# SKA-INAF/caesar-yolo

Hardware: AMD Instinct MI355X
Metric: 512x512 tiles/sec over 16k x 16k FITS (higher is better)
Workload: dtype f16

## Files before the change

caesar_yolo_amd/csrc/conv_igemm.hip:

```cpp
#include "cy_kernels.h"
#include <cmath>
#include <cstdlib>
#include <cstring>
#include <vector>

namespace cy {

typedef _Float16 f16;
typedef f16 f16x8 __attribute__((ext_vector_type(8)));
typedef f16 f16x4 __attribute__((ext_vector_type(4)));
typedef float f32x4 __attribute__((ext_vector_type(4)));
typedef unsigned int u32x4 __attribute__((ext_vector_type(4)));
typedef unsigned int u32x2 __attribute__((ext_vector_type(2)));

#define CY_OOB 0xFFFFFF00u
#define CY_WAIT_VM(N) asm volatile("s_waitcnt vmcnt(%0)" ::"n"(N) : "memory")

#ifndef CY_STAMPS_ENABLED
#define CY_STAMPS_ENABLED 0
#endif
__device__ unsigned long long g_stamps[8];
constexpr int WG_STAMP_SLOTS = 4096;
__device__ unsigned long long g_wg_stamps[WG_STAMP_SLOTS * 4];
__device__ __forceinline__ unsigned long long stamp_now() {
// ... 2649 lines not shown
        u32x4 x2[4][MI][2];
#pragma unroll
        for (int g = 0; g < 4; ++g) {
            float bv[16];
#pragma unroll
            for (int j = 0; j < 4; ++j) {
                const f32x4 t = *reinterpret_cast<const f32x4*>(bias1_lds + g * 64 + fq * 16 + j * 4);
                bv[j * 4] = t[0]; bv[j * 4 + 1] = t[1]; bv[j * 4 + 2] = t[2]; bv[j * 4 + 3] = t[3];
            }
#pragma unroll
            for (int mi = 0; mi < MI; ++mi) {
                float v[16];
                bias_act16(acc[g * 4][mi], acc[g * 4 + 1][mi], acc[g * 4 + 2][mi], acc[g * 4 + 3][mi], bv, a.act != 0, v);
                f16x8 h0, h1;
#pragma unroll
                for (int j = 0; j < 8; ++j) { h0[j] = (f16)v[j]; h1[j] = (f16)v[8 + j]; }
                x2[g][mi][0] = __builtin_bit_cast(u32x4, h0); x2[g][mi][1] = __builtin_bit_cast(u32x4, h1);
            }
        }
#pragma unroll
        for (int ni = 0; ni < NB * 4; ++ni)
#pragma unroll
            for (int mi = 0; mi < MI; ++mi) acc[ni][mi] = f32x4{0.f, 0.f, 0.f, 0.f};
        CY_WAIT_VM(0);
        __builtin_amdgcn_s_barrier();
#pragma unroll
        for (int c2 = 0; c2 < 4; ++c2) compute_x(c2, x2[c2]);
#pragma unroll
        for (int g = 0; g < NB; ++g) {
            const int cbase = g * 64 + fq * 16;
            if (cbase >= pad64(a.cout2)) continue;
            float bv[16];
#pragma unroll
            for (int j = 0; j < 4; ++j) {
                const f32x4 t = *reinterpret_cast<const f32x4*>(bias2_lds + g * 64 + fq * 16 + j * 4);
                bv[j * 4] = t[0]; bv[j * 4 + 1] = t[1]; bv[j * 4 + 2] = t[2]; bv[j * 4 + 3] = t[3];
            }
#pragma unroll
            for (int mi = 0; mi < MI; ++mi) {
                const int m = m0 + (wave * MI + mi) * 16 + fr;
                if (m >= M) continue;
                const int b = m / HoWo, r = m - b * HoWo;
                const long opix = (long)b * a.out_bs + a.out_ro + r;
                float v[16];
                bias_act16(acc[g * 4][mi], acc[g * 4 + 1][mi], acc[g * 4 + 2][mi], acc[g * 4 + 3][mi], bv, a.act2 != 0, v);
                f16* dst = reinterpret_cast<f16*>(a.out2) + opix * a.out2_ct + a.out2_coff + cbase;
                if (cbase + 16 <= a.cout2) {
                    f16x8 o0, o1;
#pragma unroll
                    for (int j = 0; j < 8; ++j) { o0[j] = (f16)v[j]; o1[j] = (f16)v[8 + j]; }
                    *reinterpret_cast<f16x8*>(dst) = o0;
                    *reinterpret_cast<f16x8*>(dst + 8) = o1;
                } else {
#pragma unroll
                    for (int j = 0; j < 16; ++j)
                        if (cbase + j < a.cout2) dst[j] = (f16)v[j];
                }
            }
        }
        return;
    }
#pragma unroll
    for (int g = 0; g < NB; ++g) {
        const int cbase = n0 + g * 64 + fq * 16;
        if (cbase >= pad64(a.Cout)) continue;
        float bv[16];
#pragma unroll
        for (int j = 0; j < 4; ++j) {
            const f32x4 t = *reinterpret_cast<const f32x4*>(bias_lds + g * 64 + fq * 16 + j * 4);
            bv[j * 4] = t[0]; bv[j * 4 + 1] = t[1]; bv[j * 4 + 2] = t[2]; bv[j * 4 + 3] = t[3];
        }
        float sc[SPLIT ? 16 : 1];
        if constexpr (SPLIT) {
#pragma unroll
            for (int j = 0; j < 16; ++j) sc[j] = a.oscale[cbase + j];
        }
#pragma unroll
        for (int mi = 0; mi < MI; ++mi) {
            const int m = m0 + (wave * MI + mi) * 16 + fr;
            if (m >= M) continue;
            const int b = m / HoWo, r = m - b * HoWo;
            const long opix = (long)b * a.out_bs + a.out_ro + r;
            float v[16];
            if constexpr (SPLIT) {
                scale_bias_act16(acc[g * 4][mi], acc[g * 4 + 1][mi], acc[g * 4 + 2][mi], acc[g * 4 + 3][mi], bv, sc, a.act != 0, v);
                f16* dst = reinterpret_cast<f16*>(a.out) + opix * a.out_ct + a.out_coff + cbase;
                const f16* rp = a.res ? reinterpret_cast<const f16*>(a.res) + (long)m * a.res_ct + a.res_coff + cbase : nullptr;
                if (cbase + 16 <= a.Cout) {
                    if (rp) {
                        const f16x8 r0v = *reinterpret_cast<const f16x8*>(rp), r1v = *reinterpret_cast<const f16x8*>(rp + 8);
                        const f16x8 q0v = *reinterpret_cast<const f16x8*>(rp + a.res_lo), q1v = *reinterpret_cast<const f16x8*>(rp + a.res_lo + 8);
#pragma unroll
                        for (int j = 0; j < 8; ++j) { v[j] += (float)r0v[j] + (float)q0v[j]; v[8 + j] += (float)r1v[j] + (float)q1v[j]; }
                    }
                    store_split16(dst, a.out_lo, v);
                } else {
#pragma unroll
                    for (int j = 0; j < 16; ++j) {
                        if (cbase + j >= a.Cout) continue;
                        float t = v[j];
                        if (rp) t += (float)rp[j] + (float)rp[a.res_lo + j];
                        store_split1(dst + j, a.out_lo, t);
                    }
                }
                continue;
            }
            bias_act16(acc[g * 4][mi], acc[g * 4 + 1][mi], acc[g * 4 + 2][mi], acc[g * 4 + 3][mi], bv, a.act != 0, v);
            if (cbase + 16 <= a.Cout) {
                f16* dst = reinterpret_cast<f16*>(a.out) + opix * a.out_ct + a.out_coff + cbase;
                if (a.res) {
                    const f16* rp = reinterpret_cast<const f16*>(a.res) + (long)m * a.res_ct + a.res_coff + cbase;
                    const f16x8 r0v = *reinterpret_cast<const f16x8*>(rp), r1v = *reinterpret_cast<const f16x8*>(rp + 8);
#pragma unroll
                    for (int j = 0; j < 8; ++j) { v[j] += (float)r0v[j]; v[8 + j] += (float)r1v[j]; }
                }
                f16x8 o0, o1;
#pragma unroll
                for (int j = 0; j < 8; ++j) { o0[j] = (f16)v[j]; o1[j] = (f16)v[8 + j]; }
                *reinterpret_cast<f16x8*>(dst) = o0;
                *reinterpret_cast<f16x8*>(dst + 8) = o1;
            } else {
#pragma unroll
                for (int j = 0; j < 16; ++j) {
                    const int c = cbase + j;
                    if (c >= a.Cout) continue;
                    float t = v[j];
                    if (a.res) t += (float)(reinterpret_cast<const f16*>(a.res)[(long)m * a.res_ct + a.res_coff + c]);
                    reinterpret_cast<f16*>(a.out)[opix * a.out_ct + a.out_coff + c] = (f16)t;
                }
            }
        }
    }
    if (stamps && tid == 0) {
        unsigned long long* rec = g_wg_stamps + (size_t)(blockIdx.x % WG_STAMP_SLOTS) * 4;
        rec[0] = t_loop - t_entry; rec[1] = t_epi - t_loop; rec[2] = stamp_real() - t_epi; rec[3] = c_epi - c_loop;
    }
}

template <int NB, int MI, int RING, bool K3, bool SPLIT = false, int NDW = 8, bool FUSE2 = false>
static hipError_t launch_direct(const ConvArgs& a, hipStream_t s) {
    constexpr int BN = 64 * NB, BM = 8 * MI * 16;
    const size_t lds = (FUSE2 ? 4 : RING) * BN * 128 + 2048;
    static bool attr_set = false;
    if (!attr_set) {
        hipFuncSetAttribute(reinterpret_cast<const void*>(conv1x1_direct_kernel<NB, MI, RING, K3, SPLIT, NDW, FUSE2>), hipFuncAttributeMaxDynamicSharedMemorySize, (int)lds);
        attr_set = true;
    }
    const int M = a.B * a.Ho * a.Wo;
    const int blocks = ((M + BM - 1) / BM) * ((pad64(a.Cout) + BN - 1) / BN);
    hipLaunchKernelGGL((conv1x1_direct_kernel<NB, MI, RING, K3, SPLIT, NDW, FUSE2>), dim3(blocks), dim3(512), lds, s, a);
    return hipGetLastError();
}

template <int WM, int RING, int PB = 2>
static hipError_t launch_halo(const ConvArgs& a, hipStream_t s) {
    constexpr int TH = 4 * WM, NT = WM * 128;
    constexpr int PR = (TH + 2) * 18, NWI = (PR + 7) / 8, NW = NT / 64, PROUNDS = (NWI + NW - 1) / NW;
    const size_t lds = PB * PROUNDS * NW * 1024 + RING * 128 * 128;
    static bool attr_set = false;
    if (!attr_set) {
        hipFuncSetAttribute(reinterpret_cast<const void*>(conv3x3_halo_kernel<WM, RING, PB>), hipFuncAttributeMaxDynamicSharedMemorySize, (int)lds);
        attr_set = true;
    }
    const int blocks = a.B * ((a.Hi + TH - 1) / TH) * ((a.Wi + 15) / 16) * ((pad64(a.Cout) + 127) / 128);
    hipLaunchKernelGGL((conv3x3_halo_kernel<WM, RING, PB>), dim3(blocks), dim3(NT), lds, s, a);
    return hipGetLastError();
}

template <typename T, int WM, int WN, int MI, int NSTAGE = 2, bool SPLIT = false>
static hipError_t launch_t(const ConvArgs& a, hipStream_t s) {
    constexpr int BM = WM * MI * 16, BN = WN * 64;
    const int M = a.B * a.Ho * a.Wo;
    const int ntm = (M + BM - 1) / BM, ntn = (pad64(a.Cout) + BN - 1) / BN;
    const size_t lds = NSTAGE * (BM + BN) * 128;
    static bool attr_set = false;
    if (!attr_set) {
        hipFuncSetAttribute(reinterpret_cast<const void*>(conv_igemm_kernel<T, WM, WN, MI, NSTAGE, SPLIT>),
                            hipFuncAttributeMaxDynamicSharedMemorySize, (int)lds);
        attr_set = true;
    }
    hipLaunchKernelGGL((conv_igemm_kernel<T, WM, WN, MI, NSTAGE, SPLIT>), dim3(ntm * ntn), dim3(WM * WN * 64), lds, s, a);
    return hipGetLastError();
}

static int head_rows(const ConvArgs& a) { const int c = a.Cout < 16 ? a.Cout : 16; const int g = (c + 3) / 4; return 16 * (g < 4 ? g : 4); }
static bool head_direct(const ConvArgs& a, int passes) {
    if (!env_knob("CY_HEAD_DIRECT", 1)) return false;
    if (!(a.k == 1 && a.s == 1 && a.c1 == 0 && !a.up0 && a.Cin >= 64 && a.Cin % 64 == 0 && a.c0 == a.Cin && pad64(a.Cout) == 64 && a.Ho == a.Hi && a.Wo == a.Wi))
        return false;
    if (a.out_f32 ? (a.res || a.act) : (a.out_bs != a.Ho * a.Wo || a.out_ro != 0 || !env_knob("CY_NARROW_DIRECT", 1))) return false;
    return (size_t)passes * (a.Cin / 64) * head_rows(a) * 128 <= 65536;
}
template <bool SPLIT>
static hipError_t launch_head(const ConvArgs& a, hipStream_t s) {
    const int nrows = head_rows(a);
    const size_t lds = (size_t)(SPLIT ? a.split : 1) * (a.Cin / 64) * nrows * 128 + (a.Cout == 64 && a.out_f32 ? 4 * 32 * 68 * 4 : 0);
    static bool attr_set = false;
    if (!attr_set) {
        hipFuncSetAttribute(reinterpret_cast<const void*>(head1x1_kernel<SPLIT>), hipFuncAttributeMaxDynamicSharedMemorySize, 65536 + 4 * 32 * 68 * 4);
        attr_set = true;
    }
    const long M = (long)a.B * a.Ho * a.Wo;
    const long wgs = (M + 127) / 128;
    hipLaunchKernelGGL((head1x1_kernel<SPLIT>), dim3((unsigned)(wgs < 512 ? wgs : 512)), dim3(256), lds, s, a, nrows);
    return hipGetLastError();
}

static int head_pair_pitch(int rowlen) { int tp = rowlen; while (tp % 8 != 4) ++tp; return tp; }
static size_t head_pair_lds(Precision p, const ConvArgs& a, const ConvArgs& b) {
    const size_t pa = p == PREC_F16X3 ? a.split : 1, pb = p == PREC_F16X3 ? b.split : 1;
    return pa * (a.Cin / 64) * 64 * 128 + pb * (b.Cin / 64) * head_rows(b) * 128 + (size_t)8 * 16 * head_pair_pitch(a.out_ct) * 4;
}
bool head_pair_ok(Precision p, const ConvArgs& a, const ConvArgs& b) {
    if (p == PREC_F32 || !env_knob("CY_HEAD_PAIR", 1)) return false;
    if (conv_variant(p, a) != CONV_HEAD_1X1 || conv_variant(p, b) != CONV_HEAD_1X1) return false;
    if (a.B != b.B || a.Ho != b.Ho || a.Wo != b.Wo || a.out != b.out || a.out_ct != b.out_ct || a.out_bs != b.out_bs || a.out_ro != b.out_ro) return false;
    if (a.out_coff != 0 || a.Cout != 64 || b.out_coff != 64 || b.Cout < 1 || b.Cout != a.out_ct - 64) return false;
    return head_pair_lds(p, a, b) <= 128 * 1024;
}
hipError_t launch_head_pair(Precision p, const ConvArgs& a, const ConvArgs& b, hipStream_t s) {
    const size_t lds = head_pair_lds(p, a, b);
    static bool attr_set = false;
    if (!attr_set) {
        hipFuncSetAttribute(reinterpret_cast<const void*>(head1x1_pair_kernel<false>), hipFuncAttributeMaxDynamicSharedMemorySize, 128 * 1024);
        hipFuncSetAttribute(reinterpret_cast<const void*>(head1x1_pair_kernel<true>), hipFuncAttributeMaxDynamicSharedMemorySize, 128 * 1024);
        attr_set = true;
    }
    const long M = (long)a.B * a.Ho * a.Wo;
    const long wgs = (M + 255) / 256;
    const unsigned grid = (unsigned)(wgs < 256 ? wgs : 256);
    if (p == PREC_F16X3) hipLaunchKernelGGL((head1x1_pair_kernel<true>), dim3(grid), dim3(512), lds, s, a, b, head_rows(b), head_pair_pitch(a.out_ct));
    else hipLaunchKernelGGL((head1x1_pair_kernel<false>), dim3(grid), dim3(512), lds, s, a, b, head_rows(b), head_pair_pitch(a.out_ct));
    return hipGetLastError();
}

static const char* const kVariantNames[CONV_NUM_VARIANTS] = {
    "conv_igemm_kernel<2,2,4> generic 128x128", "conv_igemm_kernel<4,1,2> generic 128x64",
    "conv3x3_halo2_kernel 3x3 s1 16x16px x128ch (halo<2,2> for odd slab counts)", "conv3x3_pp_kernel<2> 3x3 s1 16x16px x64ch",
    "conv3x3_pp_kernel<4> 3x3 s1 16x16px x128ch", "conv3x3_halo_kernel<4,*> 3x3 s1 16x16px x128ch",
    "conv3x3_c64_kernel<64|32> 3x3 s1 persistent, Cin 64 or 32", "conv_igemm_kernel<4,2,4,3> generic 256x128, 3-slab ring",
    "conv3x3_wide_kernel 3x3 s1 16x32px x128ch, K slabs of 32",
    "conv1x1_direct_kernel<4,2> 1x1 256px x256ch, pixels to regs", "conv1x1_direct_kernel<2,2> 1x1 256px x128ch, pixels to regs",
    "conv3x3_wide_kernel<WN=1> 3x3 s1 16x32px x64ch", "conv3x3_wide_kernel<dual> 3x3 s1 2 images x 16x16px x128ch",
    "conv3x3_widep_kernel<strip> 3x3 s1 512 flattened px x128ch, persistent",
    "head1x1_kernel detect-head output 1x1, weights stationary in LDS, fp32 rows"};
const char* conv_variant_name(int v) { return v >= 0 && v < CONV_NUM_VARIANTS ? kVariantNames[v] : "?"; }

static bool s2_direct() { static const int v = getenv("CY_S2_DIRECT") ? atoi(getenv("CY_S2_DIRECT")) : 1; return v != 0; }

bool batch_invariant() { const char* e = getenv("CY_BATCH_INVARIANT"); return !e || atoi(e) != 0; }

static int conv_variant_x3(const ConvArgs& a) {
    const bool narrow = pad64(a.Cout) <= 64;
    if (a.k == 3 && a.s == 1 && a.c1 == 0 && !a.up0 && !a.out_f32 && a.Cin % 64 == 0 && a.wgt32 && a.out_bs == a.Ho * a.Wo && a.out_ro == 0) {
        const int wpad = (a.Wi + 31) / 32 * 32;
        const bool fits = (wpad - a.Wi) * 8 <= a.Wi;
        if (narrow && a.Wi % 32 == 0) return CONV_WIDE_64;
        if (narrow && a.Cin >= 128 && env_knob("CY_STRIP", 1) && strip_small(a) && strip_fits(a)) return CONV_STRIP_128;
        if (!narrow && env_knob("CY_STRIP", 1) && strip_fits(a) && strip_cover(a.Hi, a.Wi) + 0.04 < wide2d_cover(a.Hi, a.Wi)) return CONV_STRIP_128;
        if (!narrow && fits) return CONV_WIDE_128;
        if (!narrow && a.Wi <= 16 && a.Wi >= 14) return CONV_WIDE_DUAL;
    }
    if (!a.out_f32 && a.Cin % 64 == 0 && !narrow &&
        ((a.k == 1 && a.s == 1 && (a.c1 == 0 || a.c0 % 64 == 0)) || (a.k == 3 && a.s == 2 && a.c1 == 0 && !a.up0)))
        return pad64(a.Cout) >= 256 ? CONV_DIRECT_256 : CONV_DIRECT_128;
    if (head_direct(a, a.split)) return CONV_HEAD_1X1;
    return narrow ? CONV_GENERIC_64 : CONV_GENERIC_128;
}

int conv_variant(Precision p, const ConvArgs& a) {
    if (p == PREC_F16X3) return conv_variant_x3(a);
    const bool narrow = pad64(a.Cout) <= 64;
    const long Bv = batch_invariant() && a.B < 256 ? 256 : a.B;
    if (p == PREC_F16 && a.k == 3 && a.s == 1 && a.c1 == 0 && !a.up0 && !a.out_f32 && a.Cin == 32 && narrow && a.wgt32 &&
        a.out_bs == a.Ho * a.Wo && a.out_ro == 0)
        return CONV_C64_PERSIST;
    if (p == PREC_F16 && a.k == 3 && a.s == 1 && a.c1 == 0 && !a.up0 && !a.out_f32 && a.Cin % 64 == 0 &&
        a.out_bs == a.Ho * a.Wo && a.out_ro == 0) {
        static const int force = getenv("CY_HALO_WM") ? atoi(getenv("CY_HALO_WM")) : 0;
        static const int wide64 = getenv("CY_WIDE64") ? atoi(getenv("CY_WIDE64")) : 1;
        if (narrow && wide64 && a.wgt32 && a.Cin >= 128 && a.Wi % 32 == 0 && force == 0 &&
            Bv * ((a.Hi + 15) / 16) * (a.Wi / 32) >= 256)
            return CONV_WIDE_64;
        if (narrow && force == 0 && a.wgt32 && a.Cin >= 128 && env_knob("CY_STRIP", 1) && strip_small(a) && strip_fits(a)) return CONV_STRIP_128;
        if (narrow && a.Cin == 64 && force != 8) return force == 9 ? CONV_GENERIC_64 : CONV_C64_PERSIST;
        if (narrow) return force == 9 ? CONV_GENERIC_64 : CONV_PP_64;
        if (force == 5) return CONV_PP_128;
        if (force == 4 || force == 43) return CONV_HALO16_128;
        static const int wide = getenv("CY_WIDE") ? atoi(getenv("CY_WIDE")) : 1;
        const int strip = env_knob("CY_STRIP", 1);
        if (wide && strip && a.wgt32 && strip_fits(a) && strip_cover(a.Hi, a.Wi) + 0.04 < wide2d_cover(a.Hi, a.Wi) &&
            (strip > 1 || strip_small(a) || Bv * (long)(a.Hi + 1) * (a.Wi + 1) / 512 * ((pad64(a.Cout) + 127) / 128) >= 200))
            return CONV_STRIP_128;
        const int wpad = (a.Wi + 31) / 32 * 32;
        if (wide && a.wgt32 && (wpad - a.Wi) * 8 <= a.Wi) return CONV_WIDE_128;
        const int dual = getenv("CY_WIDE_DUAL") ? atoi(getenv("CY_WIDE_DUAL")) : 1;
        if (wide && dual && a.wgt32 && a.Wi <= 16 && a.Wi >= 14 &&
            ((Bv + 1) / 2) * ((a.Hi + 15) / 16) * ((pad64(a.Cout) + 127) / 128) >= (dual > 1 ? 1 : 224))
            return CONV_WIDE_DUAL;
        return CONV_HALO8_128;
    }
    if (p == PREC_F16 && head_direct(a, 1)) return CONV_HEAD_1X1;
    if (narrow) return CONV_GENERIC_64;
    if (p == PREC_F16 && !a.out_f32 && a.Cin % 64 == 0 &&
        ((a.k == 1 && a.s == 1 && (a.c1 == 0 || a.c0 % 64 == 0)) || (a.k == 3 && a.s == 2 && a.c1 == 0 && !a.up0 && (a.Cin >= 128 || pad64(a.Cout) < 256) && s2_direct()))) {
        const char* e = getenv("CY_DIRECT_MIN_BLOCKS");
        const long min_blocks = e ? atol(e) : 256;
        static const int bn_force = getenv("CY_DIRECT_BN") ? atoi(getenv("CY_DIRECT_BN")) : 0;
        const int bn = bn_force == 128 && a.k == 1 ? 128 : (pad64(a.Cout) >= 256 ? 256 : 128);
        const long blocks = ((Bv * a.Ho * a.Wo + 255) / 256) * ((pad64(a.Cout) + bn - 1) / bn);
        if (min_blocks >= 0 && blocks >= min_blocks) return bn == 256 ? CONV_DIRECT_256 : CONV_DIRECT_128;
    }
    static const int big = getenv("CY_BIG") ? atoi(getenv("CY_BIG")) : 1;
    const long M = Bv * a.Ho * a.Wo;
    if (p == PREC_F16 && big && (M / 256) * ((pad64(a.Cout) + 127) / 128) >= big * 256) return CONV_GENERIC_BIG;
    return CONV_GENERIC_128;
}

hipError_t launch_conv(Precision p, const ConvArgs& a, hipStream_t s) {
    if (p == PREC_F16X3) {
        if ((a.split != 2 && a.split != 3) || !a.oscale) return hipErrorInvalidValue;
        switch (conv_variant_x3(a)) {
            case CONV_WIDE_128:
                if (env_knob("CY_X3_PERSIST", 0) && a.Cout % 16 == 0) return launch_widep(a, s);
                return launch_wide<2, false, 2, true>(a, s);
            case CONV_STRIP_128: return launch_strip(a, s);
            case CONV_WIDE_64: return launch_wide<1, false, 2, true>(a, s);
            case CONV_WIDE_DUAL: return launch_wide<2, true, 2, true>(a, s);
            case CONV_DIRECT_256: return a.k == 3 ? launch_direct<4, 2, 3, true, true>(a, s) : launch_direct<4, 2, 3, false, true>(a, s);
            case CONV_DIRECT_128: return a.k == 3 ? launch_direct<2, 4, 2, true, true>(a, s) : launch_direct<2, 2, 2, false, true>(a, s);
            case CONV_HEAD_1X1: return launch_head<true>(a, s);
            case CONV_GENERIC_64: return launch_t<f16, 4, 1, 2, 2, true>(a, s);
            default: return launch_t<f16, 2, 2, 4, 2, true>(a, s);
        }
    }
    switch (conv_variant(p, a)) {
        case CONV_C64_PERSIST: return a.Cin == 32 ? launch_c64<32>(a, s) : launch_c64<64>(a, s);
        case CONV_PP_64: return launch_pp<2>(a, s);
        case CONV_PP_128: { ConvArgs b2 = a; b2.dbg = dev_knob("CY_DBG", 0); return launch_pp<4>(b2, s); }
        case CONV_HALO16_128: return (getenv("CY_HALO_WM") && atoi(getenv("CY_HALO_WM")) == 43) ? launch_halo<4, 3>(a, s) : launch_halo<4, 2>(a, s);
        case CONV_HALO8_128: {
            ConvArgs b2 = a; b2.dbg = dev_knob("CY_DBG", 0);
            static const int v = getenv("CY_HALO_V") ? atoi(getenv("CY_HALO_V")) : 2;
            if (v == 2 && (a.Cin / 64) % 2 == 0) return launch_halo2(b2, s);
            return v == 1 ? launch_halo<2, 3, 1>(b2, s) : launch_halo<2, 2>(b2, s);
        }
        case CONV_GENERIC_BIG: return launch_t<f16, 4, 2, 4, 3>(a, s);
        case CONV_WIDE_128: {
            static const int tps = getenv("CY_WIDE_TPS") ? atoi(getenv("CY_WIDE_TPS")) : 2;
            ConvArgs b2 = a; b2.dbg = dev_knob("CY_DBG", 0);
            if (const int mf = env_knob("CY_WIDE_MFMA", 16); mf >= 32) return mf == 33 ? launch_wide32<1>(b2, s) : launch_wide32<0>(b2, s);
            const int wp = env_knob("CY_WIDE_PERSIST", 1);
            const long patches = (long)a.B * ((a.Wi + 31) / 32) * ((a.Hi + 15) / 16) * ((pad64(a.Cout) + 127) / 128);
            if (wp && tps == 2 && a.Cout % 16 == 0 && (wp > 1 || (patches >= 512 && a.Cin <= 128))) return launch_widep(b2, s);
            if (tps == 2 && env_knob("CY_WIDE_SCHED", 0)) return launch_wide<2, false, 2, false, 1>(b2, s);
            return tps == 3 ? launch_wide<2, false, 3>(b2, s) : launch_wide<2>(b2, s);
        }
        case CONV_STRIP_128: return launch_strip(a, s);
        case CONV_WIDE_64: return launch_wide<1>(a, s);
        case CONV_WIDE_DUAL: return launch_wide<2, true>(a, s);
        case CONV_DIRECT_256: {
            ConvArgs a2 = a; a2.dbg = dev_knob("CY_DBG", 0);
            static const int v256 = getenv("CY_D256_V") ? atoi(getenv("CY_D256_V")) : 0;
            if (a.k != 3 && v256 > 0 && a.Cin <= v256) return launch_direct<4, 1, 2, false>(a, s);
            static const int ndw = env_knob("CY_DIRECT_NDW", 0);
            if (a.wgt2 && pad64(a.Cout) == 256 && a.c1 == 0 && !a.res && !a.out_f32)
                return a.k == 3 ? launch_direct<4, 2, 3, true, false, 4, true>(a2, s) : launch_direct<4, 2, 3, false, false, 8, true>(a2, s);
            if (a.k == 3) return ndw == 8 ? launch_direct<4, 2, 3, true>(a2, s) : launch_direct<4, 2, 3, true, false, 4>(a2, s);
            return ndw == 4 ? launch_direct<4, 2, 3, false, false, 4>(a2, s) : launch_direct<4, 2, 3, false>(a2, s);
        }
        case CONV_DIRECT_128:
            if (a.k != 3 && !(getenv("CY_D128_V") && atoi(getenv("CY_D128_V")) == 0)) return launch_direct<2, 2, 2, false>(a, s);
            return a.k == 3 ? launch_direct<2, 4, 2, true>(a, s) : launch_direct<2, 2, 4, false>(a, s);
        case CONV_HEAD_1X1: return launch_head<false>(a, s);
        case CONV_GENERIC_64: return p == PREC_F16 ? launch_t<f16, 4, 1, 2>(a, s) : launch_t<float, 4, 1, 2>(a, s);
        default: return p == PREC_F16 ? launch_t<f16, 2, 2, 4>(a, s) : launch_t<float, 2, 2, 4>(a, s);
    }
}

void debug_read_wg_stamps(unsigned long long* out, int n) {
    hipDeviceSynchronize();
    hipMemcpyFromSymbol(out, HIP_SYMBOL(g_wg_stamps), (size_t)(n < WG_STAMP_SLOTS ? n : WG_STAMP_SLOTS) * 4 * sizeof(unsigned long long));
}

void debug_read_stamps(unsigned long long* out8, bool reset) {
    hipDeviceSynchronize();
    hipMemcpyFromSymbol(out8, HIP_SYMBOL(g_stamps), 8 * sizeof(unsigned long long));
    if (CY_STAMPS_ENABLED && out8[6] == 0) {
        static unsigned long long rec[WG_STAMP_SLOTS * 4];
        hipMemcpyFromSymbol(rec, HIP_SYMBOL(g_wg_stamps), sizeof(rec));
        for (int i = 0; i < WG_STAMP_SLOTS; ++i)
            if (rec[i * 4 + 1]) { out8[6] += 1; for (int j = 0; j < 4; ++j) out8[j] += rec[i * 4 + j]; }
        out8[4] = out8[0] + out8[1] + out8[2] + out8[3];
        if (reset) { memset(rec, 0, sizeof(rec)); hipMemcpyToSymbol(HIP_SYMBOL(g_wg_stamps), rec, sizeof(rec)); }
    }
    if (reset) { unsigned long long z[8] = {0}; hipMemcpyToSymbol(HIP_SYMBOL(g_stamps), z, sizeof(z)); }
}

size_t packed_weight_bytes(Precision p, int cout, int cin, int k, int chunk_bytes) {
    const int epb = chunk_bytes / (p == PREC_F16 ? 2 : 4);
    return (size_t)((cin + epb - 1) / epb) * k * k * pad128(cout) * chunk_bytes;
}

void pack_weights(Precision p, const float* W, int cout, int cin, int k, void* dst, int chunk_bytes) {
    const int taps = k * k, cp = pad128(cout), epb = chunk_bytes / (p == PREC_F16 ? 2 : 4), chunks = (cin + epb - 1) / epb;
    memset(dst, 0, packed_weight_bytes(p, cout, cin, k, chunk_bytes));
    for (int row = 0; row < cp; ++row) {
        const int blk = row >> 6, ni = (row >> 4) & 3, rr = row & 15;
        const int n = blk * 64 + (rr >> 2) * 16 + ni * 4 + (rr & 3);
        if (n >= cout) continue;
        for (int t = 0; t < taps; ++t)
            for (int c = 0; c < cin; ++c) {
                const float v = W[((size_t)n * cin + c) * taps + t];
                const size_t o = (((size_t)(c / epb) * taps + t) * cp + row) * epb + (c % epb);
                if (p == PREC_F16) reinterpret_cast<f16*>(dst)[o] = (f16)v;
                else reinterpret_cast<float*>(dst)[o] = v;
            }
    }
    (void)chunks;
}

void pack_weights_fused2(const float* W2, int cout2, int cin2, void* dst) {
    std::vector<float> perm((size_t)cout2 * cin2);
    for (int n = 0; n < cout2; ++n)
        for (int p = 0; p < cin2; ++p) {
            const int c = p >> 6, kk = (p >> 5) & 1, q = (p >> 3) & 3, j = p & 7;
            perm[(size_t)n * cin2 + p] = W2[(size_t)n * cin2 + 64 * c + 16 * q + 8 * kk + j];
        }
    pack_weights(PREC_F16, perm.data(), cout2, cin2, 1, dst);
}

int x3_passes(const float* W, int cout, int cin, int k, const float* scale) {
    const size_t per = (size_t)cin * k * k;
    for (int n = 0; n < cout; ++n) {
        const float sc = scale ? scale[n] : 1.0f;
        if (!(sc != 0.0f) || !std::isfinite(sc)) return 3;
        for (size_t i = 0; i < per; ++i) {
            const float w = W[(size_t)n * per + i];
            const f16 h = (f16)(w / sc);
            if (!((float)h * sc == w)) return 3;
        }
    }
    return 2;
}

size_t packed_weight_bytes_x3(int cout, int cin, int k, int chunk_bytes, int passes) {
    const int epb = chunk_bytes / 2;
    return packed_weight_bytes(PREC_F16, cout, passes * ((cin + epb - 1) / epb * epb), k, chunk_bytes);
}

void pack_weights_x3(const float* W, int cout, int cin, int k, void* dst, float* oscale, int chunk_bytes, int passes, const float* scale) {
    const int taps = k * k, epb = chunk_bytes / 2, cinp = (cin + epb - 1) / epb * epb, cp = pad128(cout);
    memset(dst, 0, packed_weight_bytes_x3(cout, cin, k, chunk_bytes, passes));
    for (int i = 0; i < cp; ++i) oscale[i] = 1.0f;
    f16* o = reinterpret_cast<f16*>(dst);
    for (int row = 0; row < cp; ++row) {
        const int blk = row >> 6, ni = (row >> 4) & 3, rr = row & 15;
        const int n = blk * 64 + (rr >> 2) * 16 + ni * 4 + (rr & 3);
        if (n >= cout) continue;
        if (passes == 2) {
            const float sc = scale ? scale[n] : 1.0f;
            oscale[n] = sc;
            for (int t = 0; t < taps; ++t)
                for (int c = 0; c < cin; ++c) {
                    const f16 h = (f16)(W[((size_t)n * cin + c) * taps + t] / sc);
                    for (int pass = 0; pass < 2; ++pass) {
                        const int cv = pass * cinp + c;
                        o[(((size_t)(cv / epb) * taps + t) * cp + row) * epb + (cv % epb)] = h;
                    }
                }
            continue;
        }
        float m = 0.0f;
        for (size_t i = 0; i < (size_t)cin * taps; ++i) m = fmaxf(m, fabsf(W[(size_t)n * cin * taps + i]));
        int e = 0;
        if (m > 0.0f && std::isfinite(m)) { int ex; frexpf(m, &ex); e = 14 - ex; }
        if (e > 60) e = 60;
        if (e < -60) e = -60;
        const float up = ldexpf(1.0f, e);
        oscale[n] = ldexpf(1.0f, -e);
        for (int t = 0; t < taps; ++t)
            for (int c = 0; c < cin; ++c) {
                const float v = W[((size_t)n * cin + c) * taps + t] * up;
                const f16 hi = (f16)v, lo = (f16)(v - (float)hi);
                for (int pass = 0; pass < 3; ++pass) {
                    const int cv = pass * cinp + c;
                    o[(((size_t)(cv / epb) * taps + t) * cp + row) * epb + (cv % epb)] = pass == 1 ? lo : hi;
                }
            }
    }
}

__global__ __launch_bounds__(256) void x3_split_kernel(const float* __restrict__ in, f16* __restrict__ out, long n, int C) {
    for (long i = (long)blockIdx.x * 256 + threadIdx.x; i < n; i += (long)gridDim.x * 256) {
        const long pix = i / C; const int c = (int)(i - pix * C);
        store_split1(out + pix * 2 * C + c, C, in[i]);
    }
}
__global__ __launch_bounds__(256) void x3_merge_kernel(const f16* __restrict__ in, float* __restrict__ out, long n, int C) {
    for (long i = (long)blockIdx.x * 256 + threadIdx.x; i < n; i += (long)gridDim.x * 256) {
        const long pix = i / C; const int c = (int)(i - pix * C);
        out[i] = (float)in[pix * 2 * C + c] + (float)in[pix * 2 * C + C + c];
    }
}
hipError_t launch_x3_split(const float* in, void* out, long npix, int C, hipStream_t s) {
    const long n = npix * C;
    hipLaunchKernelGGL(x3_split_kernel, dim3((unsigned)((n + 255) / 256 < 65535 ? (n + 255) / 256 : 65535)), dim3(256), 0, s, in, reinterpret_cast<f16*>(out), n, C);
    return hipGetLastError();
}
hipError_t launch_x3_merge(const void* in, float* out, long npix, int C, hipStream_t s) {
    const long n = npix * C;
    hipLaunchKernelGGL(x3_merge_kernel, dim3((unsigned)((n + 255) / 256 < 65535 ? (n + 255) / 256 : 65535)), dim3(256), 0, s, reinterpret_cast<const f16*>(in), out, n, C);
    return hipGetLastError();
}

template <typename T, bool SPLIT = false>
__global__ __launch_bounds__(256) void stem_kernel(const StemArgs a) {
    __shared__ float w[27 * 64];
    __shared__ float bs[64];
    const int co_blocks = a.Cout / 16;
    for (int i = threadIdx.x; i < 27 * a.Cout; i += 256) w[i] = a.w[i];
    for (int i = threadIdx.x; i < a.Cout; i += 256) bs[i] = a.bias[i];
    __syncthreads();
    const long total = (long)a.B * a.Ho * a.Wo * co_blocks;
    for (long idx = (long)blockIdx.x * 256 + threadIdx.x; idx < total; idx += (long)gridDim.x * 256) {
        const int cb = (int)(idx % co_blocks);
        const long pix = idx / co_blocks;
// ... 630 lines not shown
```

caesar_yolo_amd/csrc/cy_kernels.h:

```cpp
#pragma once
#include <hip/hip_runtime.h>
#include <stdint.h>
#include <stdlib.h>

namespace cy {

#ifndef CY_DEV_KNOBS
#define CY_DEV_KNOBS 0
#endif
inline int env_knob(const char* name, int dflt) { const char* e = getenv(name); return e ? atoi(e) : dflt; }
inline int dev_knob(const char* name, int dflt) { return CY_DEV_KNOBS ? env_knob(name, dflt) : dflt; }

enum Precision { PREC_F16 = 0, PREC_F32 = 1, PREC_F16X3 = 2 };

struct ConvArgs {
    const void* in0; int in0_ct, in0_coff, c0, up0;
    const void* in1; int in1_ct, in1_coff, c1;
    const void* wgt;
    const void* wgt32; uint32_t wgt32_bytes;
    const float* bias;
    void* out; int out_ct, out_coff;
    int out_bs, out_ro;
    int out_f32;
    const void* res; int res_ct, res_coff;
    int B, Hi, Wi, Ho, Wo, Cin, Cout, k, s, act;
    uint32_t in0_bytes, in1_bytes, wgt_bytes;
    int dbg;
    int split, in0_lo, in1_lo, out_lo, res_lo;
    const float* oscale;
    const void* wgt2; uint32_t wgt2_bytes; const float* bias2; int act2, cout2;
    void* out2; int out2_ct, out2_coff;
};

struct StemArgs {
    const void* in; void* out; const float* w; const float* bias;
    const void* wpk;
    int B, Hi, Wi, Ho, Wo, Cout, out_ct, out_coff;
    int out_lo;
};

struct StemDownArgs {
    const void* in; uint32_t in_bytes; int B, Hi, Wi;
    const void* wpk2; const float* bias0;
    const void* wgt32; uint32_t wgt32_bytes; const float* bias1;
    void* out; int out_ct, out_coff;
    int H1, W1, Ho, Wo;
    int dbg;
};

struct BneckArgs {
    const void* in; int in_ct, in_coff; uint32_t in_bytes;
    void* out; int out_ct, out_coff;
    const void* wfrag;
    const float* bias1; const float* bias2;
    int B, H, W, shortcut;
    int dbg;
};
constexpr size_t BNECK_WFRAG_BYTES = 2 * 4 * 18 * 1024;
hipError_t launch_bneck64(const BneckArgs& a, hipStream_t s);
void pack_bneck_weights(const float* W1, const float* W2, void* dst);

struct PoolArgs {
    const void* src; void* dst; int ct, src_coff, dst_coff, C, B, H, W;
    int lo;
};

struct DwArgs {
    const void* in; int in_ct, in_coff; void* out; int out_ct, out_coff; const void* res; int res_ct, res_coff;
    const float* w; const float* bias; int B, H, W, C, act;
    int blk, gstride, goff;
    int in_lo, out_lo, res_lo;
    int xcd;
};
struct AttnArgs {
    const void* qkv; int ct, coff; void* out; int out_ct, out_coff; int B, N, heads, kd, hd; float scale;
    int lo, out_lo;
};
hipError_t launch_dwconv(Precision p, const DwArgs& a, hipStream_t s);
hipError_t launch_attention(Precision p, const AttnArgs& a, hipStream_t s);

hipError_t launch_conv(Precision p, const ConvArgs& a, hipStream_t s);
enum ConvVariant { CONV_GENERIC_128 = 0, CONV_GENERIC_64, CONV_HALO8_128, CONV_PP_64, CONV_PP_128, CONV_HALO16_128, CONV_C64_PERSIST, CONV_GENERIC_BIG, CONV_WIDE_128, CONV_DIRECT_256, CONV_DIRECT_128, CONV_WIDE_64, CONV_WIDE_DUAL, CONV_STRIP_128, CONV_HEAD_1X1, CONV_NUM_VARIANTS };
int conv_variant(Precision p, const ConvArgs& a);
const char* conv_variant_name(int v);
bool head_pair_ok(Precision p, const ConvArgs& a, const ConvArgs& b);
hipError_t launch_head_pair(Precision p, const ConvArgs& a, const ConvArgs& b, hipStream_t s);
void debug_read_stamps(unsigned long long* out8, bool reset);
void debug_read_wg_stamps(unsigned long long* out, int n);
void debug_read_pre_stamps(unsigned long long* out8, bool reset);
void debug_fastdiv(const double* d_a, const double* d_b, double* d_fast, double* d_ref, int n);
hipError_t launch_stem(Precision p, const StemArgs& a, hipStream_t s);
hipError_t launch_stem_down(const StemDownArgs& a, hipStream_t s);
long stem_down_blocks(const StemDownArgs& a);
bool batch_invariant();
void pack_stem_weights2(const float* W, int cout, void* dst);
hipError_t launch_pool5(Precision p, const PoolArgs& a, hipStream_t s);

size_t packed_weight_bytes(Precision p, int cout, int cin, int k, int chunk_bytes = 128);
void pack_weights(Precision p, const float* W, int cout, int cin, int k, void* dst, int chunk_bytes = 128);
void pack_weights_fused2(const float* W2, int cout2, int cin2, void* dst);
int x3_passes(const float* W, int cout, int cin, int k, const float* scale);
size_t packed_weight_bytes_x3(int cout, int cin, int k, int chunk_bytes = 128, int passes = 3);
void pack_weights_x3(const float* W, int cout, int cin, int k, void* dst, float* oscale, int chunk_bytes = 128, int passes = 3, const float* scale = nullptr);
hipError_t launch_x3_split(const float* in, void* out, long npix, int C, hipStream_t s);
hipError_t launch_x3_merge(const void* in, float* out, long npix, int C, hipStream_t s);
void pack_stem_weights(const float* W, int cout, void* dst);
__device__ __forceinline__ int xcd_contiguous(int bid, int nwg) {
    const int q = nwg >> 3, r = nwg & 7, x = bid & 7;
    return (x < r ? x * (q + 1) : r * (q + 1) + (x - r) * q) + (bid >> 3);
}
__host__ __device__ inline int pad64(int c) { return (c + 63) / 64 * 64; }
__host__ __device__ inline int pad128(int c) { return (c + 127) / 128 * 128; }

struct DecodeArgs {
    const float* pred;
    int B, A, nc;
    int lvl_h[3], lvl_w[3];
    float conf;
    float* cand;
    int* cand_anchor;
    int* cand_count;
    int cap;
};
hipError_t launch_decode(const DecodeArgs& a, hipStream_t s);

struct NmsArgs {
    const float* cand; const int* cand_anchor; const int* cand_count; int cap;
    int B; float iou; int max_det;
    float gain; int padw, padh, w0, h0;
    float* det;
    int* det_anchor;
    int* det_count;
    uint64_t* keys;
    uint64_t* mask;
    int* counters;
};
hipError_t launch_nms(const NmsArgs& a, hipStream_t s);

struct MergeArgs {
    const float* det; const int* det_count; int B, max_det;
    float score_thr; double soft, hard;
    float* out; int* out_count; int* out_src;
    int* err;
    int* counters;
};
hipError_t launch_iou_merge(const MergeArgs& a, hipStream_t s);
hipError_t launch_compact_records(const float* g, long long rows, const long long* perm, int T, int stride, int* hdr, float* out, hipStream_t s);

enum PreOp { OP_BKG = 1, OP_SHIFT = 2, OP_CLIP = 3, OP_ZSCALE = 4, OP_HISTEQ = 5, OP_MINMAX = 6 };
struct PreStage { int op; double p0, p1, p2; int flag; };
constexpr int MAX_STAGES = 8;
constexpr int MAX_PRE_BATCH = 256;
struct PreProgram { int n; PreStage st[MAX_STAGES]; };
struct PreArgs {
    const float* mosaic; int MH, MW;
    int txy[2 * 256];
    int B, th, tw;
    PreProgram prog[3]; int nprog;
    double* params;
    double* histeq;
    int* status;
    void* out; int out_prec; int H, W, top, left;
    double* scratch;
    int new_h, new_w;
    int* counters;
    int variant;
    int fuse01;
};
hipError_t launch_preproc(const PreArgs& a, hipStream_t s);
hipError_t launch_preproc_planes(const PreArgs& a, hipStream_t s);
hipError_t launch_letterbox_pack(const PreArgs& a, hipStream_t s);
hipError_t launch_mosaic_prepare(float* data, size_t n, int big_endian, hipStream_t s);

}
```

Before: 8949.

## Add persistent weight-stationary 1x1 conv kernel for 128-channel outputs

Adds a persistent 1x1 convolution kernel that loads the whole filter (up to 128 KB) into LDS once per workgroup, then streams 32-pixel groups per wave through a 4-deep register prefetch ring of buffer loads and MFMAs. It replaces the direct 128-channel 1x1 kernel when Cout is 128 with no residual or split, which removes repeated weight reloads per tile. In exchange, large LDS use limits occupancy to one workgroup per CU, and the grid is capped at the CU count.

```diff
diff --git a/caesar_yolo_amd/csrc/conv_igemm.hip b/caesar_yolo_amd/csrc/conv_igemm.hip
--- a/caesar_yolo_amd/csrc/conv_igemm.hip
+++ b/caesar_yolo_amd/csrc/conv_igemm.hip
@@ -2825,6 +2825,126 @@
     return hipGetLastError();
 }
 
+constexpr int WS_MAX_FILTER = 128 * 1024;
+__global__ __launch_bounds__(512) void conv1x1_ws_kernel(const ConvArgs a) {
+    constexpr int MI = 2, PG = 16 * MI, D = 4, NW = 8, NI = 8;
+    extern __shared__ __attribute__((aligned(16))) char smem[];
+    const int tid = threadIdx.x, lane = tid & 63, wave = tid >> 6, fr = lane & 15, fq = lane >> 4;
+    const int HoWo = a.Ho * a.Wo, M = a.B * HoWo;
+    const int vch = a.Cin / 64;
+    float* const bias_lds = reinterpret_cast<float*>(smem + vch * 128 * 128);
+
+    for (int i = tid; i < vch * 128 * 8; i += NW * 64) {
+        const int q = i & 7, rr = i >> 3, r = rr & 127, cc = rr >> 7;
+        const u32x4 w = *reinterpret_cast<const u32x4*>(reinterpret_cast<const char*>(a.wgt) + ((size_t)cc * 128 + r) * 128 + q * 16);
+        *reinterpret_cast<u32x4*>(smem + (cc * 128 + r) * 128 + ((q ^ (r & 7)) << 4)) = w;
+    }
+    if (tid < 128) bias_lds[tid] = a.bias[tid];
+    __syncthreads();
+
+    const auto rs0 = __builtin_amdgcn_make_buffer_rsrc(const_cast<void*>(a.in0), 0, a.in0_bytes, 0x00020000);
+    const int ngrp = (M + PG - 1) / PG, stride = gridDim.x * NW;
+
+    u32x4 x[D][MI][2];
+    int gi = blockIdx.x * NW + wave, vi = 0;
+    auto issue = [&](u32x4 (&xs)[MI][2]) {
+        if (gi >= ngrp) return;
+#pragma unroll
+        for (int mi = 0; mi < MI; ++mi) {
+            const int m = gi * PG + mi * 16 + fr;
+            const unsigned base = (unsigned)(m * a.in0_ct + a.in0_coff + vi * 64 + fq * 8) * 2;
+#pragma unroll
+            for (int kk = 0; kk < 2; ++kk) xs[mi][kk] = load_b128(rs0, m < M ? base + kk * 64 : CY_OOB, 0);
+        }
+        if (++vi == vch) { vi = 0; gi += stride; }
+    };
+
+    f32x4 acc[NI][MI];
+#pragma unroll
+    for (int ni = 0; ni < NI; ++ni)
+#pragma unroll
+        for (int mi = 0; mi < MI; ++mi) acc[ni][mi] = f32x4{0.f, 0.f, 0.f, 0.f};
+
+    int g = gi, v = 0;
+    auto step = [&](u32x4 (&xc)[MI][2], u32x4 (&xn)[MI][2]) {
+        issue(xn);
+        const char* Wl = smem + v * 128 * 128;
+#pragma unroll
+        for (int kk = 0; kk < 2; ++kk) {
+            const int qf = fq + 4 * kk;
+#pragma unroll
+            for (int ni = 0; ni < NI; ++ni) {
+                const int r = ni * 16 + fr;
+                const f16x8 wb = *reinterpret_cast<const f16x8*>(Wl + r * 128 + ((qf ^ (r & 7)) << 4));
+#pragma unroll
+                for (int mi = 0; mi < MI; ++mi)
+                    acc[ni][mi] = __builtin_amdgcn_mfma_f32_16x16x32_f16(wb, __builtin_bit_cast(f16x8, xc[mi][kk]), acc[ni][mi], 0, 0, 0);
+            }
+        }
+        if (++v < vch) return;
+        v = 0;
+#pragma unroll
+        for (int gb = 0; gb < 2; ++gb) {
+            const int cbase = gb * 64 + fq * 16;
+            float bv[16];
+#pragma unroll
+            for (int j = 0; j < 4; ++j) {
+                const f32x4 t = *reinterpret_cast<const f32x4*>(bias_lds + cbase + j * 4);
+                bv[j * 4] = t[0]; bv[j * 4 + 1] = t[1]; bv[j * 4 + 2] = t[2]; bv[j * 4 + 3] = t[3];
+            }
+#pragma unroll
+            for (int mi = 0; mi < MI; ++mi) {
+                const int m = g * PG + mi * 16 + fr;
+                float o[16];
+                bias_act16(acc[gb * 4][mi], acc[gb * 4 + 1][mi], acc[gb * 4 + 2][mi], acc[gb * 4 + 3][mi], bv, a.act != 0, o);
+#pragma unroll
+                for (int ni = 0; ni < 4; ++ni) acc[gb * 4 + ni][mi] = f32x4{0.f, 0.f, 0.f, 0.f};
+                if (m >= M) continue;
+                const int b = m / HoWo, r = m - b * HoWo;
+                f16* dst = reinterpret_cast<f16*>(a.out) + ((long)b * a.out_bs + a.out_ro + r) * a.out_ct + a.out_coff + cbase;
+                f16x8 o0, o1;
+#pragma unroll
+                for (int j = 0; j < 8; ++j) { o0[j] = (f16)o[j]; o1[j] = (f16)o[8 + j]; }
+                *reinterpret_cast<f16x8*>(dst) = o0;
+                *reinterpret_cast<f16x8*>(dst + 8) = o1;
+            }
+        }
+        g += stride;
+    };
+
+#pragma unroll
+    for (int d = 0; d < D - 1; ++d) issue(x[d]);
+    while (true) {
+        if (g >= ngrp) break;
+        step(x[0], x[3]);
+        if (g >= ngrp) break;
+        step(x[1], x[0]);
+        if (g >= ngrp) break;
+        step(x[2], x[1]);
+        if (g >= ngrp) break;
+        step(x[3], x[2]);
+    }
+}
+
+static bool ws1x1_ok(const ConvArgs& a) {
+    if (!env_knob("CY_WS_1X1", 1)) return false;
+    return a.k == 1 && a.s == 1 && a.c1 == 0 && !a.up0 && !a.res && !a.out_f32 && !a.split && a.Cout == 128 && a.Cin % 64 == 0 &&
+           a.c0 == a.Cin && a.Ho == a.Hi && a.Wo == a.Wi && (size_t)(a.Cin / 64) * 128 * 128 <= (size_t)WS_MAX_FILTER;
+}
+static hipError_t launch_ws1x1(const ConvArgs& a, hipStream_t s) {
+    const size_t lds = (size_t)(a.Cin / 64) * 128 * 128 + 512;
+    static bool attr_set = false;
+    if (!attr_set) {
+        hipFuncSetAttribute(reinterpret_cast<const void*>(conv1x1_ws_kernel), hipFuncAttributeMaxDynamicSharedMemorySize, WS_MAX_FILTER + 512);
+        attr_set = true;
+    }
+    static const int ncu = [] { int dev = 0, n = 256; hipGetDevice(&dev); hipDeviceGetAttribute(&n, hipDeviceAttributeMultiprocessorCount, dev); return n > 0 ? n : 256; }();
+    const long M = (long)a.B * a.Ho * a.Wo;
+    const long wgs = (M + 255) / 256;
+    hipLaunchKernelGGL(conv1x1_ws_kernel, dim3((unsigned)(wgs < ncu ? wgs : ncu)), dim3(512), lds, s, a);
+    return hipGetLastError();
+}
+
 template <int WM, int RING, int PB = 2>
 static hipError_t launch_halo(const ConvArgs& a, hipStream_t s) {
     constexpr int TH = 4 * WM, NT = WM * 128;
@@ -2916,7 +3036,8 @@
     "conv1x1_direct_kernel<4,2> 1x1 256px x256ch, pixels to regs", "conv1x1_direct_kernel<2,2> 1x1 256px x128ch, pixels to regs",
     "conv3x3_wide_kernel<WN=1> 3x3 s1 16x32px x64ch", "conv3x3_wide_kernel<dual> 3x3 s1 2 images x 16x16px x128ch",
     "conv3x3_widep_kernel<strip> 3x3 s1 512 flattened px x128ch, persistent",
-    "head1x1_kernel detect-head output 1x1, weights stationary in LDS, fp32 rows"};
+    "head1x1_kernel detect-head output 1x1, weights stationary in LDS, fp32 rows",
+    "conv1x1_ws_kernel 1x1 32px x128ch per wave, weights stationary in LDS, persistent"};
 const char* conv_variant_name(int v) { return v >= 0 && v < CONV_NUM_VARIANTS ? kVariantNames[v] : "?"; }
 
 static bool s2_direct() { static const int v = getenv("CY_S2_DIRECT") ? atoi(getenv("CY_S2_DIRECT")) : 1; return v != 0; }
@@ -2982,7 +3103,7 @@
         static const int bn_force = getenv("CY_DIRECT_BN") ? atoi(getenv("CY_DIRECT_BN")) : 0;
         const int bn = bn_force == 128 && a.k == 1 ? 128 : (pad64(a.Cout) >= 256 ? 256 : 128);
         const long blocks = ((Bv * a.Ho * a.Wo + 255) / 256) * ((pad64(a.Cout) + bn - 1) / bn);
-        if (min_blocks >= 0 && blocks >= min_blocks) return bn == 256 ? CONV_DIRECT_256 : CONV_DIRECT_128;
+        if (min_blocks >= 0 && blocks >= min_blocks) return bn == 256 ? CONV_DIRECT_256 : ws1x1_ok(a) ? CONV_WS_128 : CONV_DIRECT_128;
     }
     static const int big = getenv("CY_BIG") ? atoi(getenv("CY_BIG")) : 1;
     const long M = Bv * a.Ho * a.Wo;
@@ -3046,6 +3167,7 @@
             if (a.k != 3 && !(getenv("CY_D128_V") && atoi(getenv("CY_D128_V")) == 0)) return launch_direct<2, 2, 2, false>(a, s);
             return a.k == 3 ? launch_direct<2, 4, 2, true>(a, s) : launch_direct<2, 2, 4, false>(a, s);
         case CONV_HEAD_1X1: return launch_head<false>(a, s);
+        case CONV_WS_128: return launch_ws1x1(a, s);
         case CONV_GENERIC_64: return p == PREC_F16 ? launch_t<f16, 4, 1, 2>(a, s) : launch_t<float, 4, 1, 2>(a, s);
         default: return p == PREC_F16 ? launch_t<f16, 2, 2, 4>(a, s) : launch_t<float, 2, 2, 4>(a, s);
     }
diff --git a/caesar_yolo_amd/csrc/cy_kernels.h b/caesar_yolo_amd/csrc/cy_kernels.h
--- a/caesar_yolo_amd/csrc/cy_kernels.h
+++ b/caesar_yolo_amd/csrc/cy_kernels.h
@@ -80,7 +80,7 @@
 hipError_t launch_attention(Precision p, const AttnArgs& a, hipStream_t s);
 
 hipError_t launch_conv(Precision p, const ConvArgs& a, hipStream_t s);
-enum ConvVariant { CONV_GENERIC_128 = 0, CONV_GENERIC_64, CONV_HALO8_128, CONV_PP_64, CONV_PP_128, CONV_HALO16_128, CONV_C64_PERSIST, CONV_GENERIC_BIG, CONV_WIDE_128, CONV_DIRECT_256, CONV_DIRECT_128, CONV_WIDE_64, CONV_WIDE_DUAL, CONV_STRIP_128, CONV_HEAD_1X1, CONV_NUM_VARIANTS };
+enum ConvVariant { CONV_GENERIC_128 = 0, CONV_GENERIC_64, CONV_HALO8_128, CONV_PP_64, CONV_PP_128, CONV_HALO16_128, CONV_C64_PERSIST, CONV_GENERIC_BIG, CONV_WIDE_128, CONV_DIRECT_256, CONV_DIRECT_128, CONV_WIDE_64, CONV_WIDE_DUAL, CONV_STRIP_128, CONV_HEAD_1X1, CONV_WS_128, CONV_NUM_VARIANTS };
 int conv_variant(Precision p, const ConvArgs& a);
 const char* conv_variant_name(int v);
 bool head_pair_ok(Precision p, const ConvArgs& a, const ConvArgs& b);
```

Measured after the change: 8966 (median of 6 runs). No clear change (+0.2%).
